# HIRO-group/torque_constrained_motion_planning

Hardware: NVIDIA B200
Metric: torque-feasibility states/sec (Panda 7-DOF RNE) (higher is better)
Workload: dtype f64

## Files before the change

### torque_constrained_motion_planning_b200/build.py

```python
from __future__ import annotations

import os
import shutil
import subprocess
import sys
from concurrent.futures import ThreadPoolExecutor

HERE = os.path.dirname(os.path.abspath(__file__))
CSRC = os.path.join(HERE, "csrc")
LIB = os.path.join(HERE, "libtcmp.so")
SOURCES = ["rne_kernels.cu", "model_kernels.cu", "edge_kernels.cu", "ik_kernels.cu", "select_kernels.cu", "collision_kernels.cu", "dynamics_kernels.cu", "tcmp_api.cu"]
HEADERS = ["panda_model.cuh", "collision_core.cuh", "dynamics_core.cuh", "ik_core.cuh", "sincos_table.inc", "tcmp_internal.h", os.path.join("..", "..", "include", "tcmp.h")]

NVCC_FLAGS = [
    "-gencode", "arch=compute_100a,code=sm_100a",
    "-O3", "-std=c++17", "-lineinfo", "--expt-relaxed-constexpr",
    "-Xcompiler", "-fPIC,-O2",
    "-Xptxas", "-v",
]


def _nvcc() -> str:
    for cand in (os.environ.get("NVCC"), "/usr/local/cuda/bin/nvcc", shutil.which("nvcc")):
        if cand and os.path.exists(cand):
            return cand
    raise RuntimeError("nvcc not found")


def _stale() -> bool:
    if not os.path.exists(LIB):
        return True
    t = os.path.getmtime(LIB)
    deps = [os.path.join(CSRC, s) for s in SOURCES + HEADERS] + [os.path.abspath(__file__)]
    return any(os.path.getmtime(d) > t for d in deps if os.path.exists(d))


SOURCE_FLAGS = {}


def build(force: bool = False, verbose: bool = False, defines=(), suffix: str = "", source_flags=None) -> str:
    per_source = dict(SOURCE_FLAGS)
    per_source.update(source_flags or {})
    lib_path = LIB if not suffix else os.path.join(HERE, "libtcmp%s.so" % suffix)
    if not force and not suffix and not _stale():
        return LIB
    nvcc = _nvcc()
    objdir = os.path.join(HERE, "build" + suffix)
    os.makedirs(objdir, exist_ok=True)
    env = dict(os.environ)
    ccbin = "/usr/bin/g++" if os.path.exists("/usr/bin/g++") else shutil.which("g++")

    def compile_one(src):
        obj = os.path.join(objdir, src.replace(".cu", ".o"))
        cmd = [nvcc, "-ccbin", ccbin, *NVCC_FLAGS, *per_source.get(src, []), *["-D" + d for d in defines], "-c",
               os.path.join(CSRC, src), "-o", obj]
        r = subprocess.run(cmd, capture_output=True, text=True, env=env)
        log = r.stdout + r.stderr
        with open(os.path.join(objdir, src + ".ptxas.log"), "w") as f:
            f.write(log)
        if r.returncode != 0:
            raise RuntimeError("nvcc failed for %s:\n%s" % (src, log))
        if verbose:
            print(log)
        return obj

    with ThreadPoolExecutor(max_workers=len(SOURCES)) as ex:
        objs = list(ex.map(compile_one, SOURCES))
    cmd = [nvcc, "-ccbin", ccbin, "-shared", "-gencode", "arch=compute_100a,code=sm_100a", "-o", lib_path, *objs]
    r = subprocess.run(cmd, capture_output=True, text=True, env=env)
    if r.returncode != 0:
        raise RuntimeError("link failed:\n" + r.stdout + r.stderr)
    return lib_path


if __name__ == "__main__":
    print(build(force="--force" in sys.argv, verbose="--verbose" in sys.argv))
```

### torque_constrained_motion_planning_b200/csrc/rne_kernels.cu

```cuda
#include "panda_model.cuh"
#include "tcmp_internal.h"

namespace tcmp {

#ifndef TCMP_PDL
#define TCMP_PDL 1
#endif
#ifndef TCMP_INT_INDEX
#define TCMP_INT_INDEX 1
#endif
#ifndef TCMP_RNE_WAVES
#define TCMP_RNE_WAVES 4
#endif
#ifndef TCMP_DOUBLE_BUFFER
#define TCMP_DOUBLE_BUFFER 1
#endif
#if TCMP_DOUBLE_BUFFER && !defined(TCMP_RNE_MIN_BLOCKS)
#define TCMP_RNE_MIN_BLOCKS 3
#endif

#ifndef TCMP_TABLE_SINCOS
#define TCMP_TABLE_SINCOS 1
#endif
__device__ const SinCos kSinCosTable[kSinCosTableSize] = {
#include "sincos_table.inc"
};

struct MaskDests {
    uint8_t *p[TCMP_MAX_PEERS];
    int n;
    int64_t offset;
    uint8_t *mc;
};

struct SyncDests {
    PeerSync *sync[TCMP_MAX_PEERS];
    int n_sync, rank;
};

template <typename I>
__device__ __forceinline__ void scatter_mask(const MaskDests &dests, I at, I n, bool ok) {
    if (dests.mc) {
        const int lane = threadIdx.x & 31;
        const I base = at - (I)lane;
        if (base + 32 <= n) {
            const unsigned b = __ballot_sync(0xffffffffu, ok);
            if (lane < 2) {
                const unsigned h16 = (b >> (lane * 16)) & 0xffffu;
                auto spread = [](unsigned x) { return (x & 1u) | ((x & 2u) << 7) | ((x & 4u) << 14) | ((x & 8u) << 21); };
                const unsigned w0 = spread(h16 & 0xfu), w1 = spread((h16 >> 4) & 0xfu),
                               w2 = spread((h16 >> 8) & 0xfu), w3 = spread((h16 >> 12) & 0xfu);
                uint8_t *dst = dests.mc + dests.offset + base + lane * 16;
                asm volatile("multimem.st.relaxed.sys.global.v4.f32 [%0], {%1, %2, %3, %4};" ::"l"(dst),
                             "f"(__uint_as_float(w0)), "f"(__uint_as_float(w1)), "f"(__uint_as_float(w2)),
                             "f"(__uint_as_float(w3))
                             : "memory");
            }
            return;
        }
    }
    const uint8_t m = (uint8_t)ok;
#pragma unroll
    for (int d = 0; d < TCMP_MAX_PEERS; ++d)
        if (d < dests.n) dests.p[d][dests.offset + at] = m;
}

#ifndef TCMP_RNE_BLOCK
#define TCMP_RNE_BLOCK 128
#endif
#ifdef TCMP_RNE_MIN_BLOCKS
#define TCMP_RNE_BOUNDS TCMP_RNE_BLOCK, TCMP_RNE_MIN_BLOCKS
#else
#define TCMP_RNE_BOUNDS TCMP_RNE_BLOCK
#endif
template <typename T, typename I, bool DYN, bool TOOL, bool WRITE_TAU, bool WRITE_MASK, bool SCATTER = false>
__global__ void __launch_bounds__(TCMP_RNE_BOUNDS)
rne_batch_kernel(I n, const T *__restrict__ q, const T *__restrict__ qd, const T *__restrict__ qdd,
                 const T *__restrict__ payload_mass, T payload_scalar, T payload_threshold,
                 T *__restrict__ tau_out, uint8_t *__restrict__ feasible_out, const __grid_constant__ MaskDests dests) {
    constexpr bool kTable = TCMP_TABLE_SINCOS && sizeof(T) == 8 && DYN;
    __shared__ SinCos tab[kTable ? kSinCosTableSize : 1];
    if constexpr (kTable) {
        for (int t = threadIdx.x; t < kSinCosTableSize; t += blockDim.x) tab[t] = kSinCosTable[t];
        __syncthreads();
    }
#if TCMP_PDL
    asm volatile("griddepcontrol.launch_dependents;");
    asm volatile("griddepcontrol.wait;" ::: "memory");
#endif
#if TCMP_DOUBLE_BUFFER
    const I stride = (I)(gridDim.x * blockDim.x);
    I i = (I)(blockIdx.x * blockDim.x + threadIdx.x);
    const bool any = i < n;
    auto load = [&](I at, T (&lq)[7], T (&lv)[7], T (&la)[7], T &lm) {
#pragma unroll
        for (int j = 0; j < 7; ++j) {
            lq[j] = __ldcs(q + j * n + at);
            if constexpr (DYN) { lv[j] = __ldcs(qd + j * n + at); la[j] = __ldcs(qdd + j * n + at); }
        }
        lm = payload_mass ? __ldcs(payload_mass + at) : payload_scalar;
    };
    auto consume = [&](I at, const T (&lq)[7], const T (&lv)[7], const T (&la)[7], T lm) {
        T tau[7];
        const T mp_inertial = TOOL ? T(0) : (lm > payload_threshold ? lm : T(0));
        const T mp_tool = TOOL ? lm : T(0);
        if constexpr (kTable) rne_core_table<DYN, TOOL>(lq, lv, la, mp_inertial, mp_tool, tau, tab);
        else rne_core<T, DYN, TOOL>(lq, lv, la, mp_inertial, mp_tool, tau);
        if constexpr (WRITE_TAU) {
#pragma unroll
            for (int j = 0; j < 7; ++j) __stcs(tau_out + j * n + at, tau[j]);
        }
        if constexpr (SCATTER) {
            scatter_mask<I>(dests, at, n, within_limits<T>(tau));
        } else if constexpr (WRITE_MASK) {
            __stcs(feasible_out + at, (uint8_t)within_limits<T>(tau));
        }
    };
    if (any) {
        T qa[7], va[7], aa[7], ma, qb[7], vb[7], ab[7], mb;
        load(i, qa, va, aa, ma);
        for (;;) {
            const I nx = i + stride;
            const bool more = nx < n;
            if (more) load(nx, qb, vb, ab, mb);
            consume(i, qa, va, aa, ma);
            if (!more) break;
#pragma unroll
            for (int j = 0; j < 7; ++j) {
                qa[j] = qb[j];
                if constexpr (DYN) { va[j] = vb[j]; aa[j] = ab[j]; }
            }
            ma = mb;
            i = nx;
        }
    }
}
#else
    const I stride = (I)(gridDim.x * blockDim.x);
    for (I i = (I)(blockIdx.x * blockDim.x + threadIdx.x); i < n; i += stride) {
        T qs[7], vs[7], as[7], tau[7];
#pragma unroll
        for (int j = 0; j < 7; ++j) qs[j] = __ldcs(q + j * n + i);
        if constexpr (DYN) {
#pragma unroll
            for (int j = 0; j < 7; ++j) vs[j] = __ldcs(qd + j * n + i);
#pragma unroll
            for (int j = 0; j < 7; ++j) as[j] = __ldcs(qdd + j * n + i);
        }
        const T mass = payload_mass ? __ldcs(payload_mass + i) : payload_scalar;
        const T mp_inertial = TOOL ? T(0) : (mass > payload_threshold ? mass : T(0));
        const T mp_tool = TOOL ? mass : T(0);
        if constexpr (kTable) rne_core_table<DYN, TOOL>(qs, vs, as, mp_inertial, mp_tool, tau, tab);
        else rne_core<T, DYN, TOOL>(qs, vs, as, mp_inertial, mp_tool, tau);
        if constexpr (WRITE_TAU) {
#pragma unroll
            for (int j = 0; j < 7; ++j) __stcs(tau_out + j * n + i, tau[j]);
        }
        if constexpr (SCATTER) {
            scatter_mask<I>(dests, i, n, within_limits<T>(tau));
        } else if constexpr (WRITE_MASK) {
            __stcs(feasible_out + i, (uint8_t)within_limits<T>(tau));
        }
    }
}
#endif

static inline bool fits_int(int64_t n) { return n < (int64_t)(0x7fffffff / 7) - 148 * 32 * 2048; }

template <typename T, typename I, bool DYN, bool TOOL, bool WT, bool WM, bool SC>
static cudaError_t launch_kernel(int64_t n, const void *q, const void *qd, const void *qdd, const void *pm, double ps,
                                 double pt, void *tau, uint8_t *mask, const MaskDests &dests, cudaStream_t st) {
    auto kern = rne_batch_kernel<T, I, DYN, TOOL, WT, WM, SC>;
    const int64_t want = (n + TCMP_RNE_BLOCK - 1) / TCMP_RNE_BLOCK;
    const int64_t cap = (int64_t)grid_for(reinterpret_cast<const void *>(kern), TCMP_RNE_BLOCK, n) * TCMP_RNE_WAVES;
    const int grid = (int)(want < cap ? want : cap);
#if TCMP_PDL
    cudaLaunchConfig_t cfg = {};
    cfg.gridDim = dim3(grid);
    cfg.blockDim = dim3(TCMP_RNE_BLOCK);
    cfg.stream = st;
    cudaLaunchAttribute attr[1];
    attr[0].id = cudaLaunchAttributeProgrammaticStreamSerialization;
    attr[0].val.programmaticStreamSerializationAllowed = 1;
    cfg.attrs = attr;
    cfg.numAttrs = 1;
    return cudaLaunchKernelEx(&cfg, kern, (I)n, (const T *)q, (const T *)qd, (const T *)qdd, (const T *)pm, (T)ps,
                              (T)pt, (T *)tau, mask, dests);
#else
    kern<<<grid, TCMP_RNE_BLOCK, 0, st>>>((I)n, (const T *)q, (const T *)qd, (const T *)qdd, (const T *)pm, (T)ps,
                                          (T)pt, (T *)tau, mask, dests);
    return cudaGetLastError();
#endif
}

template <typename T, bool DYN, bool TOOL, bool WT, bool WM, bool SC>
static cudaError_t launch_indexed(int64_t n, const void *q, const void *qd, const void *qdd, const void *pm, double ps,
                                  double pt, void *tau, uint8_t *mask, const MaskDests &dests, cudaStream_t st) {
#if TCMP_INT_INDEX
    if (fits_int(n)) return launch_kernel<T, int, DYN, TOOL, WT, WM, SC>(n, q, qd, qdd, pm, ps, pt, tau, mask, dests, st);
#endif
    return launch_kernel<T, int64_t, DYN, TOOL, WT, WM, SC>(n, q, qd, qdd, pm, ps, pt, tau, mask, dests, st);
}

template <typename T, bool DYN, bool TOOL, bool WT, bool WM>
static cudaError_t launch_one(int64_t n, const void *q, const void *qd, const void *qdd, const void *pm,
                              double ps, double pt, void *tau, uint8_t *mask, cudaStream_t st) {
    MaskDests none = {};
    return launch_indexed<T, DYN, TOOL, WT, WM, false>(n, q, qd, qdd, pm, ps, pt, tau, mask, none, st);
}

template <typename T, bool DYN, bool TOOL>
static cudaError_t launch_outputs(int64_t n, const void *q, const void *qd, const void *qdd, const void *pm,
                                  double ps, double pt, void *tau, uint8_t *mask, cudaStream_t st) {
    if (tau && mask) return launch_one<T, DYN, TOOL, true, true>(n, q, qd, qdd, pm, ps, pt, tau, mask, st);
    if (tau) return launch_one<T, DYN, TOOL, true, false>(n, q, qd, qdd, pm, ps, pt, tau, mask, st);
    return launch_one<T, DYN, TOOL, false, true>(n, q, qd, qdd, pm, ps, pt, tau, mask, st);
}

template <typename T>
static cudaError_t launch_typed(int mode, int64_t n, const void *q, const void *qd, const void *qdd,
                                const void *pm, double ps, double pt, void *tau, uint8_t *mask,
                                cudaStream_t st) {
    const bool dynamic = (mode != TCMP_MODE_NOV) && qd && qdd;
    const bool tool = (mode == TCMP_MODE_DYN);
    if (dynamic) {
        if (tool) return launch_outputs<T, true, true>(n, q, qd, qdd, pm, ps, pt, tau, mask, st);
        return launch_outputs<T, true, false>(n, q, qd, qdd, pm, ps, pt, tau, mask, st);
    }
    if (tool) return launch_outputs<T, false, true>(n, q, qd, qdd, pm, ps, pt, tau, mask, st);
    return launch_outputs<T, false, false>(n, q, qd, qdd, pm, ps, pt, tau, mask, st);
}

cudaError_t launch_rne_batch(int mode, int dtype, int64_t n, const void *q, const void *qd, const void *qdd,
                             const void *pm, double ps, double pt, void *tau, uint8_t *mask,
                             cudaStream_t st) {
    if (mode == TCMP_MODE_BASE) {
        cudaError_t e = cudaSuccess;
        if (mask) e = launch_fill<uint8_t>(n, mask, 1, st);
        if (tau && e == cudaSuccess)
            e = dtype == TCMP_F64 ? launch_fill<double>(7 * n, (double *)tau, 0.0, st)
                                  : launch_fill<float>(7 * n, (float *)tau, 0.f, st);
        return e;
    }
    if (dtype == TCMP_F64) return launch_typed<double>(mode, n, q, qd, qdd, pm, ps, pt, tau, mask, st);
    return launch_typed<float>(mode, n, q, qd, qdd, pm, ps, pt, tau, mask, st);
}

template <typename T, bool DYN, bool TOOL>
static cudaError_t launch_scatter_t(int64_t n, const void *q, const void *qd, const void *qdd, const void *pm,
                                    double ps, double pt, void *tau, const MaskDests &dests, cudaStream_t st) {
    if (tau) return launch_indexed<T, DYN, TOOL, true, true, true>(n, q, qd, qdd, pm, ps, pt, tau, nullptr, dests, st);
    return launch_indexed<T, DYN, TOOL, false, true, true>(n, q, qd, qdd, pm, ps, pt, tau, nullptr, dests, st);
}

__global__ void peer_signal_kernel(SyncDests d) {
    PeerSync *own = d.sync[d.rank];
    const unsigned long long e = own->epoch + 1;
    own->epoch = e;
    __threadfence_system();
    for (int r = 0; r < d.n_sync; ++r) *reinterpret_cast<volatile unsigned long long *>(&d.sync[r]->arrived[d.rank]) = e;
}

__global__ void peer_wait_kernel(PeerSync *own, int world) {
    const unsigned long long e = own->epoch;
    if ((int)threadIdx.x < world) {
        const unsigned long long *flag = &own->arrived[threadIdx.x];
        unsigned long long v;
        const long long t0 = clock64();
        for (;;) {
            asm volatile("ld.acquire.sys.global.u64 %0, [%1];" : "=l"(v) : "l"(flag) : "memory");
            if (v >= e) break;
            if (clock64() - t0 > 40000000000ll) {
                own->pad[0] = 1u + threadIdx.x;
                break;
            }
            __nanosleep(200);
        }
    }
}

__global__ void __launch_bounds__(256)
peer_push_kernel(const uint8_t *__restrict__ src, int64_t bytes, MaskDests d, int vec) {
    const int64_t stride = (int64_t)gridDim.x * blockDim.x;
    const int64_t tid = (int64_t)blockIdx.x * blockDim.x + threadIdx.x;
    if (vec) {
        const int64_t nv = bytes / 16;
        const uint4 *s4 = reinterpret_cast<const uint4 *>(src);
        for (int64_t i = tid; i < nv; i += stride) {
            const uint4 v = __ldg(s4 + i);
#pragma unroll
            for (int r = 0; r < TCMP_MAX_PEERS; ++r)
                if (r < d.n) reinterpret_cast<uint4 *>(d.p[r] + d.offset)[i] = v;
        }
        for (int64_t i = nv * 16 + tid; i < bytes; i += stride) {
            const uint8_t v = src[i];
#pragma unroll
            for (int r = 0; r < TCMP_MAX_PEERS; ++r)
                if (r < d.n) d.p[r][d.offset + i] = v;
        }
    } else {
        for (int64_t i = tid; i < bytes; i += stride) {
            const uint8_t v = src[i];
#pragma unroll
            for (int r = 0; r < TCMP_MAX_PEERS; ++r)
                if (r < d.n) d.p[r][d.offset + i] = v;
        }
    }
}

cudaError_t launch_peer_push(const void *src, int64_t bytes, int n_dest, void *const *dests, int64_t dest_offset,
                             cudaStream_t st) {
    MaskDests d = {};
    d.n = n_dest;
    d.offset = dest_offset;
    int vec = ((uintptr_t)src % 16 == 0);
    for (int i = 0; i < n_dest; ++i) {
        d.p[i] = (uint8_t *)dests[i];
        if (((uintptr_t)dests[i] + (uintptr_t)dest_offset) % 16 != 0) vec = 0;
    }
    const int64_t units = vec ? bytes / 16 : bytes;
    int grid = (int)((units + 255) / 256);
    if (grid > 32) grid = 32;
    if (grid < 1) grid = 1;
    peer_push_kernel<<<grid, 256, 0, st>>>((const uint8_t *)src, bytes, d, vec);
    return cudaGetLastError();
}

cudaError_t launch_peer_signal(int rank, int n_dest, void *const *dest_sync, cudaStream_t st) {
    SyncDests d = {};
    d.n_sync = n_dest;
    d.rank = rank;
    for (int i = 0; i < n_dest; ++i) d.sync[i] = (PeerSync *)dest_sync[i];
    peer_signal_kernel<<<1, 1, 0, st>>>(d);
    return cudaGetLastError();
}

cudaError_t launch_peer_wait(void *own_sync, int world, cudaStream_t st) {
    peer_wait_kernel<<<1, 32, 0, st>>>((PeerSync *)own_sync, world);
    return cudaGetLastError();
}

cudaError_t launch_rne_batch_scatter(int mode, int dtype, int64_t n, const void *q, const void *qd, const void *qdd,
                                     const void *pm, double ps, double pt, void *tau, int n_dest,
                                     void *const *dest_masks, int64_t dest_offset, cudaStream_t st, void *mc_masks) {
    MaskDests d = {};
    d.n = n_dest;
    d.offset = dest_offset;
    for (int i = 0; i < TCMP_MAX_PEERS; ++i) d.p[i] = i < n_dest ? (uint8_t *)dest_masks[i] : nullptr;
    d.mc = (mc_masks && ((uintptr_t)mc_masks + (uintptr_t)dest_offset) % 16 == 0) ? (uint8_t *)mc_masks : nullptr;
    if (dtype != TCMP_F64) return cudaErrorNotSupported;
    const bool dynamic = (mode != TCMP_MODE_NOV) && qd && qdd;
    const bool tool = (mode == TCMP_MODE_DYN);
    if (mode == TCMP_MODE_BASE) {
        cudaError_t e = cudaSuccess;
        for (int i = 0; i < n_dest && e == cudaSuccess; ++i) e = launch_fill<uint8_t>(n, d.p[i] + dest_offset, 1, st);
        return e;
    }
    if (dynamic) {
        if (tool) return launch_scatter_t<double, true, true>(n, q, qd, qdd, pm, ps, pt, tau, d, st);
        return launch_scatter_t<double, true, false>(n, q, qd, qdd, pm, ps, pt, tau, d, st);
    }
    if (tool) return launch_scatter_t<double, false, true>(n, q, qd, qdd, pm, ps, pt, tau, d, st);
    return launch_scatter_t<double, false, false>(n, q, qd, qdd, pm, ps, pt, tau, d, st);
}

}
```

Measured before the change: 19.30 billion.

## Process two RNE states per thread with interleaved paired evaluation

Adds a paired path in the RNE batch kernel where each thread evaluates two states (lane and lane+32 within a warp chunk). The loads for both states are issued together and the two sin/cos table lookups and RNE bodies run back to back, which gives more independent FP64 work per thread to hide latency. The launch halves the grid per element and uses a min-blocks of 2 instead of 3, so more registers are available per thread at the cost of occupancy. An optional q-prefetch variant exists but is disabled, and the build script gains an out_dir option.

```diff
diff --git a/torque_constrained_motion_planning_b200/build.py b/torque_constrained_motion_planning_b200/build.py
--- a/torque_constrained_motion_planning_b200/build.py
+++ b/torque_constrained_motion_planning_b200/build.py
@@ -38,14 +38,16 @@
 SOURCE_FLAGS = {}
 
 
-def build(force: bool = False, verbose: bool = False, defines=(), suffix: str = "", source_flags=None) -> str:
+def build(force: bool = False, verbose: bool = False, defines=(), suffix: str = "", source_flags=None,
+          out_dir: str = None) -> str:
     per_source = dict(SOURCE_FLAGS)
     per_source.update(source_flags or {})
-    lib_path = LIB if not suffix else os.path.join(HERE, "libtcmp%s.so" % suffix)
-    if not force and not suffix and not _stale():
+    dest = out_dir or HERE
+    lib_path = LIB if not suffix and not out_dir else os.path.join(dest, "libtcmp%s.so" % suffix)
+    if not force and not suffix and not out_dir and not _stale():
         return LIB
     nvcc = _nvcc()
-    objdir = os.path.join(HERE, "build" + suffix)
+    objdir = os.path.join(dest, "build" + suffix)
     os.makedirs(objdir, exist_ok=True)
     env = dict(os.environ)
     ccbin = "/usr/bin/g++" if os.path.exists("/usr/bin/g++") else shutil.which("g++")
diff --git a/torque_constrained_motion_planning_b200/csrc/rne_kernels.cu b/torque_constrained_motion_planning_b200/csrc/rne_kernels.cu
--- a/torque_constrained_motion_planning_b200/csrc/rne_kernels.cu
+++ b/torque_constrained_motion_planning_b200/csrc/rne_kernels.cu
@@ -21,6 +21,18 @@
 
 #ifndef TCMP_TABLE_SINCOS
 #define TCMP_TABLE_SINCOS 1
+#endif
+#ifndef TCMP_RNE_PAIRS
+#define TCMP_RNE_PAIRS 1
+#endif
+#ifndef TCMP_RNE_PAIR_PREFETCH
+#define TCMP_RNE_PAIR_PREFETCH 0
+#endif
+#ifndef TCMP_RNE_PAIR_MIN_BLOCKS
+#define TCMP_RNE_PAIR_MIN_BLOCKS 2
+#endif
+#ifndef TCMP_RNE_PAIR_WAVES
+#define TCMP_RNE_PAIR_WAVES 4
 #endif
 __device__ const SinCos kSinCosTable[kSinCosTableSize] = {
 #include "sincos_table.inc"
@@ -68,17 +80,38 @@
 #ifndef TCMP_RNE_BLOCK
 #define TCMP_RNE_BLOCK 128
 #endif
+template <typename T, bool DYN> constexpr bool kRneTable = TCMP_TABLE_SINCOS && sizeof(T) == 8 && DYN;
+template <typename T, typename I, bool DYN>
+constexpr bool kRnePairs = TCMP_RNE_PAIRS && kRneTable<T, DYN> && sizeof(I) == 4;
 #ifdef TCMP_RNE_MIN_BLOCKS
-#define TCMP_RNE_BOUNDS TCMP_RNE_BLOCK, TCMP_RNE_MIN_BLOCKS
+#define TCMP_RNE_BOUNDS TCMP_RNE_BLOCK, (kRnePairs<T, I, DYN> ? TCMP_RNE_PAIR_MIN_BLOCKS : TCMP_RNE_MIN_BLOCKS)
 #else
-#define TCMP_RNE_BOUNDS TCMP_RNE_BLOCK
-#endif
+#define TCMP_RNE_BOUNDS TCMP_RNE_BLOCK, (kRnePairs<T, I, DYN> ? TCMP_RNE_PAIR_MIN_BLOCKS : 1)
+#endif
+template <bool DYN, bool TOOL>
+__device__ __forceinline__ void rne_pair_table(const double (&qa)[7], const double (&va)[7], const double (&aa)[7],
+                                               double mia, double mta, double (&ta)[7], const double (&qb)[7],
+                                               const double (&vb)[7], const double (&ab)[7], double mib, double mtb,
+                                               double (&tb)[7], const SinCos *__restrict__ tab) {
+    double sa[7], ca[7], sb[7], cb[7];
+    if (!sincos6_table(qa, sa, ca, tab)) {
+#pragma unroll
+        for (int j = 1; j < 7; ++j) sincos(qa[j], &sa[j], &ca[j]);
+    }
+    if (!sincos6_table(qb, sb, cb, tab)) {
+#pragma unroll
+        for (int j = 1; j < 7; ++j) sincos(qb[j], &sb[j], &cb[j]);
+    }
+    rne_body<double, DYN, TOOL>(sa, ca, va, aa, mia, mta, ta);
+    rne_body<double, DYN, TOOL>(sb, cb, vb, ab, mib, mtb, tb);
+}
+
 template <typename T, typename I, bool DYN, bool TOOL, bool WRITE_TAU, bool WRITE_MASK, bool SCATTER = false>
 __global__ void __launch_bounds__(TCMP_RNE_BOUNDS)
 rne_batch_kernel(I n, const T *__restrict__ q, const T *__restrict__ qd, const T *__restrict__ qdd,
                  const T *__restrict__ payload_mass, T payload_scalar, T payload_threshold,
                  T *__restrict__ tau_out, uint8_t *__restrict__ feasible_out, const __grid_constant__ MaskDests dests) {
-    constexpr bool kTable = TCMP_TABLE_SINCOS && sizeof(T) == 8 && DYN;
+    constexpr bool kTable = kRneTable<T, DYN>;
     __shared__ SinCos tab[kTable ? kSinCosTableSize : 1];
     if constexpr (kTable) {
         for (int t = threadIdx.x; t < kSinCosTableSize; t += blockDim.x) tab[t] = kSinCosTable[t];
@@ -88,6 +121,77 @@
     asm volatile("griddepcontrol.launch_dependents;");
     asm volatile("griddepcontrol.wait;" ::: "memory");
 #endif
+    if constexpr (kRnePairs<T, I, DYN>) {
+        const int lane = threadIdx.x & 31;
+        const I stride = (I)gridDim.x * (I)blockDim.x * 2;
+        I i = ((I)blockIdx.x * (I)blockDim.x + (I)(threadIdx.x & ~31u)) * 2 + (I)lane;
+        auto second = [&](I at) { return at + 32 < n ? at + 32 : at; };
+        auto load_q = [&](I at, T (&lq)[7]) {
+#pragma unroll
+            for (int j = 0; j < 7; ++j) lq[j] = __ldcs(q + j * n + at);
+        };
+        auto load_rest = [&](I at, T (&lv)[7], T (&la)[7], T &lm) {
+#pragma unroll
+            for (int j = 0; j < 7; ++j) { lv[j] = __ldcs(qd + j * n + at); la[j] = __ldcs(qdd + j * n + at); }
+            lm = payload_mass ? __ldcs(payload_mass + at) : payload_scalar;
+        };
+        auto finish = [&](I at, const T (&tau)[7]) {
+            if constexpr (WRITE_TAU) {
+#pragma unroll
+                for (int j = 0; j < 7; ++j) __stcs(tau_out + j * n + at, tau[j]);
+            }
+            if constexpr (SCATTER) {
+                scatter_mask<I>(dests, at, n, within_limits<T>(tau));
+            } else if constexpr (WRITE_MASK) {
+                __stcs(feasible_out + at, (uint8_t)within_limits<T>(tau));
+            }
+        };
+        auto eval = [&](I at, const T (&qa)[7], const T (&va)[7], const T (&aa)[7], T ma, const T (&qb)[7],
+                        const T (&vb)[7], const T (&ab)[7], T mb) {
+            T ta[7], tb[7];
+            const T mia = TOOL ? T(0) : (ma > payload_threshold ? ma : T(0)), mta = TOOL ? ma : T(0);
+            const T mib = TOOL ? T(0) : (mb > payload_threshold ? mb : T(0)), mtb = TOOL ? mb : T(0);
+            rne_pair_table<DYN, TOOL>(qa, va, aa, mia, mta, ta, qb, vb, ab, mib, mtb, tb, tab);
+            finish(at, ta);
+            if (at + 32 < n) finish(at + 32, tb);
+        };
+#if TCMP_RNE_PAIR_PREFETCH == 0
+        for (; i < n; i += stride) {
+            const I ib = second(i);
+            T qa[7], va[7], aa[7], ma, qb[7], vb[7], ab[7], mb;
+            load_q(i, qa);
+            load_q(ib, qb);
+            load_rest(i, va, aa, ma);
+            load_rest(ib, vb, ab, mb);
+            eval(i, qa, va, aa, ma, qb, vb, ab, mb);
+        }
+#else
+        if (i < n) {
+            T qa[7], qb[7];
+            load_q(i, qa);
+            load_q(second(i), qb);
+            for (;;) {
+                const I ib = second(i);
+                T va[7], aa[7], ma, vb[7], ab[7], mb;
+                load_rest(i, va, aa, ma);
+                load_rest(ib, vb, ab, mb);
+                const I nx = i + stride;
+                const bool more = nx < n;
+                T qa2[7], qb2[7];
+                if (more) {
+                    load_q(nx, qa2);
+                    load_q(second(nx), qb2);
+                }
+                eval(i, qa, va, aa, ma, qb, vb, ab, mb);
+                if (!more) break;
+#pragma unroll
+                for (int j = 0; j < 7; ++j) { qa[j] = qa2[j]; qb[j] = qb2[j]; }
+                i = nx;
+            }
+        }
+#endif
+        return;
+    }
 #if TCMP_DOUBLE_BUFFER
     const I stride = (I)(gridDim.x * blockDim.x);
     I i = (I)(blockIdx.x * blockDim.x + threadIdx.x);
@@ -165,14 +269,20 @@
 }
 #endif
 
-static inline bool fits_int(int64_t n) { return n < (int64_t)(0x7fffffff / 7) - 148 * 32 * 2048; }
+static inline bool fits_int(int64_t n) {
+    constexpr int64_t kOvershoot = 2 * (int64_t)(TCMP_RNE_WAVES > TCMP_RNE_PAIR_WAVES ? TCMP_RNE_WAVES : TCMP_RNE_PAIR_WAVES) *
+                                   148 * 2048 + 32;
+    return n < (int64_t)(0x7fffffff / 7) - kOvershoot;
+}
 
 template <typename T, typename I, bool DYN, bool TOOL, bool WT, bool WM, bool SC>
 static cudaError_t launch_kernel(int64_t n, const void *q, const void *qd, const void *qdd, const void *pm, double ps,
                                  double pt, void *tau, uint8_t *mask, const MaskDests &dests, cudaStream_t st) {
     auto kern = rne_batch_kernel<T, I, DYN, TOOL, WT, WM, SC>;
-    const int64_t want = (n + TCMP_RNE_BLOCK - 1) / TCMP_RNE_BLOCK;
-    const int64_t cap = (int64_t)grid_for(reinterpret_cast<const void *>(kern), TCMP_RNE_BLOCK, n) * TCMP_RNE_WAVES;
+    constexpr int64_t per_cta = kRnePairs<T, I, DYN> ? 2 * TCMP_RNE_BLOCK : TCMP_RNE_BLOCK;
+    constexpr int waves = kRnePairs<T, I, DYN> ? TCMP_RNE_PAIR_WAVES : TCMP_RNE_WAVES;
+    const int64_t want = (n + per_cta - 1) / per_cta;
+    const int64_t cap = (int64_t)grid_for(reinterpret_cast<const void *>(kern), TCMP_RNE_BLOCK, n) * waves;
     const int grid = (int)(want < cap ? want : cap);
 #if TCMP_PDL
     cudaLaunchConfig_t cfg = {};
```

After: 17.47 billion (median of 6 runs). -9.5%, worse.
